# NIFTy-PPL/NIFTy

Hardware: AMD Instinct MI355X
Metric: MGVI iters/sec on 1024^3 RGSpace CorrelatedField, 8 samples; achieved HBM GB/s (higher is better)
Workload: dtype f32

## Files before the change

include/niftyk.h:

```cpp
#ifndef NIFTYK_H
#define NIFTYK_H
#include <stddef.h>
#include <stdint.h>

#ifdef __cplusplus
extern "C" {
#endif

typedef enum {
  NK_OK = 0,
  NK_ERR_INVALID = -1,
  NK_ERR_UNSUPPORTED = -2,
  NK_ERR_RUNTIME = -3,
  NK_ERR_NOMEM = -4
} nk_status;

typedef enum { NK_F32 = 0, NK_F64 = 1 } nk_dtype;

#define NK_HARTLEY_NON_CANONICAL 0
#define NK_HARTLEY_CANONICAL 1

enum { NK_PRO_PLAIN = 0, NK_PRO_AMP = 1, NK_PRO_AMP_JVP = 2, NK_PRO_MUL = 3 };
enum { NK_EPI_AFFINE = 0, NK_EPI_MUL = 1, NK_EPI_VJP = 2, NK_EPI_LIKELIHOOD = 3, NK_EPI_NONLIN = 4 };
enum { NK_LH_GAUSS = 0, NK_LH_POISSON = 1 };
// ... 110 lines not shown
typedef struct nk_tiled_csr {
  int64_t n_rows, n_slots;
  int32_t n_items, ny, nx, th, tw;
  const int32_t* item_tile;
  const int64_t* item_blk;
  const int32_t* blk_slot;
  const int64_t* row_slot;
  const uint16_t* loc;
  const float* wgt;
} nk_tiled_csr;
int nk_tiled_rowsum(const nk_tiled_csr* m, int count, const void* const* x, void* const* y, double* scratch, int dtype,
                    void* stream);

int nk_roll(int ndim, const int64_t* shape, const int64_t* shift, int elem_bytes, const void* in, void* out, void* stream);

int nk_bluestein_rows(int64_t rows, int n, int m, const void* in, const void* w, const void* bhat_br, const void* tw, void* out,
                      double scale, int in_real, int out_hartley, int dtype, void* stream);

int nk_cumsum(int64_t n, const void* in, void* out, int reverse, int dtype, void* stream);

int nk_cplx_rows(int64_t rows, int64_t in_cols, int64_t out_cols, const void* a, const void* w, void* out, int mode,
                 double scale, int sgn, int dtype, void* stream);

int nk_fold_copies(int64_t n, int copies, int64_t stride, const double* src, double* dst, void* stream);

int nk_octant_expand(int ndim, const int64_t* shape, const void* table, const int32_t* pidx, void* field, int dtype,
                     int compact, void* stream);
int nk_octant_scatter(int ndim, const int64_t* shape, const double* w8, const int32_t* pidx, double* abar,
                      int merge_swapped_lines, void* stream);
int nk_octant_expand_k2(int ndim, const int64_t* shape, const double* table, const int32_t* bin_k2, int64_t nb, void* dense,
                        void* field8, int dtype, const int32_t* line_order, void* stream);
int nk_octant_scatter_k2(int ndim, const int64_t* shape, const double* w8, const int32_t* pidx, const int32_t* bin_k2,
                         int64_t nb, double* scratch, double* abar, const double* w8max, void* stream);
int nk_segment_sum(int64_t nseg, const int32_t* rowptr, const int32_t* perm, const double* src, double* dst, int accumulate,
                   void* stream);
int nk_plan_octant_vjp(const nk_plan* plan);

int nk_pindex_from_k2(int ndim, const int64_t* shape, const int32_t* k2table, int32_t* pidx, int64_t* rho,
                      void* stream);

int nk_cg_curv(int64_t n, const void* d, const void* q, int dtype, double* scal, int accumulate, void* stream);
int nk_cg_update(int64_t n, void* x, void* r, const void* d, const void* q, const void* b, int dtype,
                 double* scal, int accumulate, void* stream);
int nk_cg_update_dr(int64_t n, void* x, void* r, const void* d, const void* q, int dtype, double* scal, int accumulate,
                    void* stream);
int nk_cg_direction(int64_t n, void* d, const void* r, int dtype, double* scal, int roll, void* stream);

typedef struct nk_product {
  int nsub;
  int64_t size[3];
  const int32_t* pidx[3];
  const double* tab[3];
  const double* dtab[3];
  const double* scale;
  const double* dscale;
} nk_product;
int nk_product_field(const nk_product* p, int tangent, void* out, int dtype, void* stream);
int nk_mirror_combine(int ndim, const int64_t* shape, const int* group, int nsub, const double* coef, const void* in,
                      void* out, double scale, double offset, int dtype, void* stream);
size_t nk_product_marginal_scratch(const nk_product* p, int which);
int nk_product_marginal(const nk_product* p, int which, const double* w, double* scratch, double* marg, void* stream);

int nk_amp_forward(int nb, const double* geo, const double* hyp, const double* lat, double* state, double* amp,
                   void* stream);
int nk_amp_jvp(int nb, const double* geo, const double* hyp, const double* lat, double* state, const double* dlat,
               double* damp, void* stream);
// ... 91 lines not shown
```

nifty_amd/_lib.py:

```python
import ctypes
import os

_HERE = os.path.dirname(os.path.abspath(__file__))
LIB_PATH = os.environ.get("NK_LIB_PATH") or os.path.join(_HERE, "csrc", "libniftyk.so")

NK_OK, NK_ERR_INVALID, NK_ERR_UNSUPPORTED, NK_ERR_RUNTIME, NK_ERR_NOMEM = 0, -1, -2, -3, -4
NK_F32, NK_F64 = 0, 1
PRO_PLAIN, PRO_AMP, PRO_AMP_JVP, PRO_MUL = 0, 1, 2, 3
EPI_AFFINE, EPI_MUL, EPI_VJP, EPI_LIKELIHOOD, EPI_NONLIN = 0, 1, 2, 3, 4
LH_GAUSS, LH_POISSON = 0, 1
NL_ID, NL_EXP, NL_SIGMOID = 0, 1, 2
OP_ADD, OP_SUB, OP_MUL, OP_DIV = 0, 1, 2, 3

_vp, _i, _i64, _d, _sz = ctypes.c_void_p, ctypes.c_int, ctypes.c_int64, ctypes.c_double, ctypes.c_size_t


class Fuse(ctypes.Structure):

    _fields_ = [
        ("pro", _i), ("in_", _vp), ("in2", _vp), ("pidx", _vp), ("amp", _vp), ("damp", _vp),
        ("epi", _i), ("out", _vp), ("scale", _d), ("offset", _d), ("mul", _vp), ("mul_scalar", _d),
        ("xi", _vp), ("addend", _vp), ("addend_scale", _d), ("accumulate", _i), ("abar", _vp), ("lh_kind", _i), ("nonlin", _i), ("data", _vp),
        ("icov", _vp), ("icov_scalar", _d), ("out2", _vp), ("value", _vp),
        ("afield", _vp), ("dampT", _vp), ("abar_copies", _i), ("abar_stride", _i64), ("dafield", _vp), ("w8", _vp),
# ... 44 lines not shown
    "nk_hartley_sandwich_pair": (_i, [_vp, ctypes.POINTER(Fuse), ctypes.POINTER(Fuse), _d, _i, _vp, _vp, _vp]),
    "nk_hartley_sandwich_group": (_i, [_vp, ctypes.POINTER(Fuse), _i, _d, _i, _vp, _vp]),
    "nk_group_order": (_i, [_i64, _i, ctypes.POINTER(_i64), ctypes.POINTER(_i64)]),
    "nk_group_grid_size": (_i64, [_i64, _i]),
    "nk_fftn": (_i, [_vp, _vp, _vp, _i, _d, _vp, _vp]),
    "nk_plan_c2c_ok": (_i, [_vp]),
    "nk_plan_c2c_lds": (_i, [_vp, ctypes.POINTER(_i64)]),
    "nk_profile_enable": (_i, [_i]),
    "nk_profile_collect": (_i, [_vp, _vp]),
    "nk_vdot": (_i, [_i64, _vp, _vp, _i, _vp, _i, _vp]),
    "nk_product_field": (_i, [ctypes.POINTER(Product), _i, _vp, _i, _vp]),
    "nk_mirror_combine": (_i, [_i, ctypes.POINTER(_i64), ctypes.POINTER(_i), _i, ctypes.POINTER(_d), _vp, _vp, _d, _d, _i, _vp]),
    "nk_product_marginal_scratch": (_sz, [ctypes.POINTER(Product), _i]),
    "nk_product_marginal": (_i, [ctypes.POINTER(Product), _i, _vp, _vp, _vp, _vp]),
    "nk_red_unit": (_i64, [_i64, _i]),
    "nk_red_layout": (_i, [_i64, _i, _i, _i, _i, _i, _vp]),
    "nk_red_finish": (_i, [_vp, _i, _i, _vp, _i, _vp]),
    "nk_sum": (_i, [_i64, _vp, _i, _vp, _i, _vp]),
    "nk_stats": (_i, [_i64, _vp, _i, _vp, _vp]),
    "nk_binary": (_i, [_i, _i64, _vp, _d, _vp, _d, _vp, _i, _vp]),
    "nk_cplx_muldiv": (_i, [_i64, _vp, _i, _d, _d, _vp, _i, _d, _d, _i, _i, _vp, _i, _vp]),
    "nk_cplx_pointwise": (_i, [_i, _i64, _vp, _vp, _i, _vp]),
    "nk_axpby": (_i, [_i64, _d, _vp, _d, _vp, _vp, _i, _vp]),
    "nk_axpby_sqnorm": (_i, [_i64, _d, _vp, _d, _vp, _vp, _i, _vp, _i, _vp]),
    "nk_pointwise": (_i, [_i, _d, _i64, _vp, _vp, _vp, _i, _vp]),
    "nk_clip": (_i, [_d, _d, _i64, _vp, _vp, _vp, _i, _vp]),
    "nk_gather": (_i, [_i64, _vp, _vp, _vp, _i, _vp]),
    "nk_scatter_add": (_i, [_i64, _vp, _vp, _i64, _vp, _i, _vp]),
    "nk_octant_expand": (_i, [_i, ctypes.POINTER(_i64), _vp, _vp, _vp, _i, _i, _vp]),
    "nk_octant_scatter": (_i, [_i, ctypes.POINTER(_i64), _vp, _vp, _vp, _i, _vp]),
    "nk_octant_expand_k2": (_i, [_i, ctypes.POINTER(_i64), _vp, _vp, _i64, _vp, _vp, _i, _vp, _vp]),
    "nk_segment_sum": (_i, [_i64, _vp, _vp, _vp, _vp, _i, _vp]),
    "nk_octant_scatter_k2": (_i, [_i, ctypes.POINTER(_i64), _vp, _vp, _vp, _i64, _vp, _vp, _vp, _vp]),
    "nk_plan_octant_vjp": (_i, [_vp]),
    "nk_fold_copies": (_i, [_i64, _i, _i64, _vp, _vp, _vp]),
    "nk_cumsum": (_i, [_i64, _vp, _vp, _i, _i, _vp]),
    "nk_cplx_rows": (_i, [_i64, _i64, _i64, _vp, _vp, _vp, _i, _d, _i, _i, _vp]),
    "nk_csr_rowsum": (_i, [_i64, _vp, _vp, _vp, _vp, _vp, _i, _i, _vp]),
    "nk_tiled_rowsum": (_i, [ctypes.POINTER(TiledCsr), _i, _vp, _vp, _vp, _i, _vp]),
    "nk_bluestein_rows": (_i, [_i64, _i, _i, _vp, _vp, _vp, _vp, _vp, _d, _i, _i, _i, _vp]),
    "nk_roll": (_i, [_i, ctypes.POINTER(_i64), ctypes.POINTER(_i64), _i, _vp, _vp, _vp]),
    "nk_spmv": (_i, [_i64, _vp, _vp, _vp, _vp, _vp, _i, _vp]),
    "nk_spmv_t": (_i, [_i64, _vp, _vp, _vp, _vp, _vp, _i, _vp]),
    "nk_pindex_from_k2": (_i, [_i, ctypes.POINTER(_i64), _vp, _vp, _vp, _vp]),
    "nk_cg_curv": (_i, [_i64, _vp, _vp, _i, _vp, _i, _vp]),
    "nk_cg_update": (_i, [_i64, _vp, _vp, _vp, _vp, _vp, _i, _vp, _i, _vp]),
    "nk_cg_update_dr": (_i, [_i64, _vp, _vp, _vp, _vp, _i, _vp, _i, _vp]),
    "nk_pcg64_normal_scratch_bytes": (_i64, [_i64, _i]),
    "nk_pcg64_normal": (_i, [_vp, _vp, _i64, _d, _d, _vp, _i, _vp, _i64, _i, _vp, _vp]),
    "nk_pcg64_fixed_scratch_bytes": (_i64, []),
    "nk_pcg64_uniform": (_i, [_vp, _vp, _i64, _d, _d, _vp, _i, _vp, _vp]),
    "nk_pcg64_pm1": (_i, [_vp, _vp, _i64, _vp, _i, _i, _vp, _vp]),
    "nk_pcg64_integers_scratch_bytes": (_i64, [_i64]),
    "nk_pcg64_integers": (_i, [_vp, _vp, _i64, _i64, ctypes.c_uint64, _i64, _vp, _vp, _vp, _vp]),
    "nk_cg_direction": (_i, [_i64, _vp, _vp, _i, _vp, _i, _vp]),
    "nk_amp_forward": (_i, [_i, _vp, _vp, _vp, _vp, _vp, _vp]),
    "nk_amp_jvp": (_i, [_i, _vp, _vp, _vp, _vp, _vp, _vp, _vp]),
    "nk_amp_vjp": (_i, [_i, _vp, _vp, _vp, _vp, _vp, _vp, _vp]),
    "nk_nufft_spread": (_i, [ctypes.POINTER(NufftPlan), _vp, _vp, _vp, _i, _vp]),
    "nk_nufft_interp": (_i, [ctypes.POINTER(NufftPlan), _vp, _vp, _i, _vp]),
    "nk_nufft_crop": (_i, [ctypes.POINTER(NufftPlan), _vp, _vp, _i, _vp]),
    "nk_nufft_pad": (_i, [ctypes.POINTER(NufftPlan), _vp, _i, _vp, _i, _vp]),
    "nk_sample_times": (_i, [ctypes.POINTER(SamplePlan), _vp, _vp, _i, _vp]),
    "nk_sample_adjoint": (_i, [ctypes.POINTER(SamplePlan), _vp, _vp, _vp, _i, _vp]),
    "nk_regrid_times": (_i, [_i64, _i64, _i64, _i64, _vp, _vp, _vp, _i, _vp, _i, _vp]),
    "nk_regrid_adjoint": (_i, [_i64, _i64, _i64, _i64, _vp, _vp, _vp, _i, _vp, _i, _vp]),
# ... 66 lines not shown
```

nifty_amd/csrc/nk_vec.hip:

```cpp
#include <hip/hip_runtime.h>

#include <algorithm>
#include <cfloat>

#include <cstdint>
#include <cstdlib>
#include <type_traits>

#include "nk_core.h"
#include "nk_util.h"

static constexpr int NK_VEC_THREADS = 256;
static constexpr int NK_MAX_BLOCKS = 256 * 8;
static constexpr int NK_VEC_CHUNK = 4096;

template <typename F, typename = void>
struct NkChunkUnits {
  static constexpr int value = NK_VEC_CHUNK / NK_VEC_THREADS;
};
template <typename F>
struct NkChunkUnits<F, std::void_t<decltype(F::CHUNK_UNITS)>> {
  static constexpr int value = F::CHUNK_UNITS;
};
static inline int nk_vec_env_int(const char* name, int dflt) {
// ... 1669 lines not shown
  __syncthreads();
  const bool ok = finite && npoints < (1u << 18);
  double* dst = partial + (int64_t)s * pstride + bin0;
  for (int i = threadIdx.x; i < nbin; i += blockDim.x)
    dst[i] = ok ? (double)(long long)acc[i] * inv : __longlong_as_double(0x7ff8000000000000LL);
}

extern "C" int nk_octant_scatter_k2(int ndim, const int64_t* shape, const double* w8, const int32_t* pidx,
                                    const int32_t* bin_k2, int64_t nb, double* scratch, double* abar, const double* w8max,
                                    void* stream) {
  NkOct o;
  int rc = nk_make_oct(ndim, shape, o);
  if (rc != NK_OK) return rc;
  if (!w8 || !pidx || !bin_k2 || !scratch || !abar || nb < 1 || nb > 0x7fffffff)
    return nk_set_error(NK_ERR_INVALID, "nk_octant_scatter_k2: bad argument");
  if ((int64_t)(o.Ah - 1) * (o.Ah - 1) + (int64_t)(o.Mh - 1) * (o.Mh - 1) + (int64_t)(o.Ch - 1) * (o.Ch - 1) >= (1 << 24))
    return nk_set_error(NK_ERR_UNSUPPORTED, "nk_octant_scatter_k2: k^2 range too large");
  const int64_t shells = (nb + NK_SHELL_BINS - 1) / NK_SHELL_BINS;
  const int64_t pstride = (nb + 31) / 32 * 32;
  static const int fp_atomics = nk_vec_env_int("NK_SCATTER_FP_ATOMICS", 0);
  const bool fixed = w8max != nullptr && !fp_atomics &&
                     (int64_t)o.Ah * o.Mh * o.Ch / NK_SHELL_SPLITS < ((int64_t)1 << 16) * shells;
  if (fixed)
    hipLaunchKernelGGL(k_octant_scatter_k2_fx, dim3((unsigned)(shells * NK_SHELL_SPLITS)), dim3(256), 0, (hipStream_t)stream, o,
                       w8, pidx, bin_k2, (int)nb, pstride, scratch, w8max);
  else
    hipLaunchKernelGGL(k_octant_scatter_k2, dim3((unsigned)(shells * NK_SHELL_SPLITS)), dim3(256), 0, (hipStream_t)stream, o, w8,
                       pidx, bin_k2, (int)nb, pstride, scratch);
  rc = nk_check_launch("k_octant_scatter_k2");
  if (rc != NK_OK) return rc;
  return nk_fold_copies(nb, NK_SHELL_SPLITS, pstride, scratch, abar, stream);
}

template <typename T, int LANES>
__global__ void __launch_bounds__(256) k_csr_rowsum(int64_t nrows, const int64_t* __restrict__ rowptr,
                                                    const int32_t* __restrict__ col, const float* __restrict__ wgt,
                                                    const T* __restrict__ x, T* __restrict__ y) {
  const int64_t gid = (int64_t)blockIdx.x * blockDim.x + threadIdx.x;
  const int64_t row = gid / LANES;
  const int lane = (int)(gid % LANES);
  int64_t lo = 0, hi = 0;
  if (row < nrows) lo = rowptr[row], hi = rowptr[row + 1];
  double acc = 0.0;
  if (wgt) {
    for (int64_t j = lo + lane; j < hi; j += LANES) acc += (double)wgt[j] * (double)x[col[j]];
  } else {
    for (int64_t j = lo + lane; j < hi; j += LANES) acc += (double)x[col[j]];
  }
#pragma unroll
  for (int off = LANES / 2; off > 0; off >>= 1) acc += __shfl_down(acc, off, LANES);
  if (lane == 0 && row < nrows) y[row] = (T)acc;
}

template <typename T>
__global__ void k_spmv_t(int64_t nrows, const int64_t* __restrict__ rowptr, const int32_t* __restrict__ col,
                         const float* __restrict__ wgt, const T* __restrict__ y, double* __restrict__ x) {
  const int lane = threadIdx.x & 63;
  const int64_t row = (int64_t)blockIdx.x * (blockDim.x >> 6) + (threadIdx.x >> 6);
  if (row >= nrows) return;
  const int64_t lo = rowptr[row], hi = rowptr[row + 1];
  const double yv = (double)y[row];
  for (int64_t j = lo + lane; j < hi; j += 64) atomicAdd(x + col[j], (double)wgt[j] * yv);
}


template <int MB>
// ... 417 lines not shown
```

nifty_amd/engine.py:

```python
import contextlib
import ctypes
import math
import os
import threading

import numpy as np
import torch

from . import _lib as L
from . import backend as B
from . import batched, parallel, random
from .domains import PowerSpace, RGSpace
from .minimization import ConjugateGradient, Energy, QuadraticEnergy

SMALL_KEYS = ("asperity", "flexibility", "fluctuations", "loglogavgslope", "zeromode")
LATENT_KEYS = ("asperity", "flexibility", "fluctuations", "loglogavgslope", "spectrum", "xi", "zeromode")
_NONLIN = {None: L.NL_ID, "": L.NL_ID, "exp": L.NL_EXP, "sigmoid": L.NL_SIGMOID}
SPECTRUM_DEVICE_DRAW_MAX_POINTS = int(os.environ.get("NK_SPECTRUM_DEVICE_DRAW_MAX_POINTS", str(1 << 25)))


def lognormal_moments(mean, sigma):
    checked = {}
    for name, value in (("mean", mean), ("sig", sigma)):
        checked[name] = float(value)
# ... 230 lines not shown
        return LatentVec(B.axpby(float(a), self.xi), B.axpby(float(a), self.small))

    __rmul__ = __mul__

    def __neg__(self):
        return self * (-1.0)

    def axpy(self, a, x):
        return x._lin(float(a), self, 1.0)

    def dot_device(self, o, result=None):
        res = B.vdot(self.xi.reshape(-1), o.xi.reshape(-1), result=result, accumulate=result is not None)
        return B.vdot(self.small, o.small, result=res, accumulate=True)

    def s_vdot(self, o):
        return float(self.dot_device(o).item())

    def norm(self, ord=2):
        if ord != 2:
            raise NotImplementedError
        return math.sqrt(self.s_vdot(self))


class _Dest:

    __slots__ = ("xi", "accumulate", "carries", "small", "after", "fresh")

    def __init__(self, xi, accumulate=False, carries=(), small=None, after=(), fresh=False):
        self.xi, self.accumulate, self.carries, self.small, self.after, self.fresh = xi, accumulate, carries, small, after, fresh


class _ScratchSet:

    __slots__ = ("damp", "dafield", "w8", "w8max", "workspace")

    def __init__(self, damp, dafield, w8, w8max, workspace):
        self.damp, self.dafield, self.w8, self.w8max, self.workspace = damp, dafield, w8, w8max, workspace


class _PairTree:

    MAX_CARRIES = 2

    def __init__(self, out, scratch):
        self._stack = []
        self._first = out
        self._pool = scratch
        self._free = []

    def place(self, last, small=None):
        size, joined = 1, []
        while self._stack and (last or self._stack[-1][0] == size):
            n, t = self._stack.pop()
            joined.append(t)
            size += n
        if not joined:
            t = self._first if self._first is not None else (self._free.pop() if self._free else self._pool())
            self._first = None
            self._stack.append((1, t))
            return _Dest(t, small=small, fresh=True)
        ride = joined[:self.MAX_CARRIES] if len(joined) > 1 else []
        target = joined[len(ride)] if len(joined) > len(ride) else None
        if target is None:
            target, ride = ride[-1], ride[:-1]
        rest = joined[len(ride) + 1:]
        after, inner = [], target
        for t in rest:
            after.append((t, inner))
            inner = t
        self._free += ride + ([target] + rest[:-1] if rest else [])
# ... 76 lines not shown
            self.abar = torch.zeros(nb, dtype=torch.float64, device=self.device)
            self.damp = torch.empty(nb, dtype=torch.float64, device=self.device)
            self.latbar = torch.empty(self.nsmall, dtype=torch.float64, device=self.device)
            self.tmp = torch.empty(self.shape, dtype=dtype, device=self.device)
            self.octant_vjp = bool(L.load().nk_plan_octant_vjp(self.plan.handle))
            sw = os.environ.get("NK_SANDWICH", "1")
            self.sandwich = (self.octant_vjp and B.plan_sandwich(self.plan) and sw != "0"
                             and (len(self.shape) == 3 or sw == "2"))
            self.fused_direction = self.sandwich and os.environ.get("NK_CG_FUSED_DIRECTION", "1") != "0"
            oct_n = int(np.prod([n // 2 + 1 for n in self.shape]))
            self.field_shape = (oct_n,) if self.octant_vjp else self.shape
            self.pidx8 = None
            if self.octant_vjp:
                osl = tuple(slice(0, n // 2 + 1) for n in self.shape)
                self.pidx8 = self.pidx.view(self.shape)[osl].contiguous().reshape(-1)
            self.dafield = torch.empty(self.field_shape, dtype=dtype, device=self.device)
            self.w8 = torch.empty(oct_n, dtype=torch.float64, device=self.device) if self.octant_vjp else None
            self.w8max = torch.zeros(1, dtype=torch.float64, device=self.device)
            self.merge_swapped = int(len(self.shape) == 3 and self.shape[0] == self.shape[1]
                                     and hsp.distances[0] == hsp.distances[1])
            self.bin_k2 = None
            self.seg_plan = None
            if self.octant_vjp and len(self.shape) == 3 and ps._data.get("k2table") is not None and max(self.shape) >= 64:
                k2 = np.nonzero(hsp._k2_flags())[0].astype(np.int32)
                if len(k2) == nb and int(k2[-1]) < (1 << 24):
                    self.bin_k2 = torch.from_numpy(k2).to(self.device)
            self.scatter_fixed_point = False
            if self.bin_k2 is not None:
                a_idx = torch.arange(self.shape[0] // 2 + 1, device=self.device, dtype=torch.int64)
                key = (self.pidx8.view(self.shape[0] // 2 + 1, -1) // 4096).to(torch.int64) * 16 + (a_idx % 16)[:, None]
                self.scatter_busiest = int(torch.bincount(key.reshape(-1)).max().item())
                self.scatter_fixed_point = self.scatter_busiest < (1 << 18)
                del key, a_idx
            self.k2_dense = self.k2_line_order = None
            if self.bin_k2 is not None and os.environ.get("NK_EXPAND_K2", "1") != "0":
                self.k2_dense = torch.zeros(int(self.bin_k2[-1].item()) + 1, dtype=dtype, device=self.device)
                if len(self.shape) == 3 and os.environ.get("NK_EXPAND_ORDER", "1") != "0":
                    a2 = torch.arange(self.shape[0] // 2 + 1, device=self.device, dtype=torch.int64) ** 2
                    b2 = torch.arange(self.shape[1] // 2 + 1, device=self.device, dtype=torch.int64) ** 2
                    self.k2_line_order = torch.argsort((a2[:, None] + b2[None, :]).reshape(-1), stable=True).to(torch.int32)
            if self.octant_vjp and self.bin_k2 is None and os.environ.get("NK_SEGMENT_SUM", "1") != "0":
                self.seg_plan = B.bin_plan(self.pidx8, self.nb)
            self.wide = (dtype == torch.float32 and self.octant_vjp and os.environ.get("NK_WIDE_FORWARD", "1") != "0")
            self.wide_generic = (dtype == torch.float32 and not self.octant_vjp
                                 and os.environ.get("NK_WIDE_FORWARD", "1") != "0")
            self._wide_state = None
            if (not self.octant_vjp and self.N <= B.BIN_PLAN_MAX and os.environ.get("NK_SEGMENT_SUM", "1") != "0"):
                self.full_plan = B.bin_plan(self.pidx, self.nb)
                self.wfull = torch.empty(self.N, dtype=torch.float64, device=self.device)
        if likelihood not in ("gaussian", "poisson"):
            raise ValueError("likelihood must be 'gaussian' or 'poisson'")
        self.lh_kind = L.LH_GAUSS if likelihood == "gaussian" else L.LH_POISSON
        self.nonlin = _NONLIN[nonlin]
        self.icov_field, self.icov_scalar = None, 1.0
        self.response = response
        self.wide_response = False
        self.data_shape = self.shape if response is None else (int(response.n_data),)
        if response is not None:
            if int(response.n_pix) != self.N:
                raise ValueError("response does not act on this grid")
            if getattr(response, "grid_shape", 0) is None:
                response.grid_shape = tuple(self.shape)
            self.sandwich = self.fused_direction = False
            self.wide_response = self.wide or self.wide_generic
            self.wide = self.wide_generic = False
        if data is not None:
# ... 102 lines not shown
            f.abar, f.w8 = self.abar.data_ptr(), sc.w8.data_ptr()
            if self.scatter_fixed_point:
                f.w8max = sc.w8max.data_ptr()
        elif self.full_plan is not None:
            f.abar, f.wfull = self.abar.data_ptr(), self.wfull.data_ptr()
        else:
            f.abar, f.abar_copies, f.abar_stride = self.abar_priv.data_ptr(), self.abar_copies, self.abar_stride

    def _amp_tangent(self, lp, d, sc, gather=False):
        L.check(L.load().nk_amp_jvp(self.nb, self.geo.data_ptr(), self.hyp.data_ptr(), lp.x.small.data_ptr(),
                                    lp.state.data_ptr(), d.small.data_ptr(), sc.damp.data_ptr(), B._stream()), "nk_amp_jvp")
        if gather:
            return sc.damp if self.tdtype == torch.float64 else sc.damp.to(self.tdtype)
        self._amp_field(sc.damp, out=sc.dafield)

    def _bin_sums(self, sc):
        shp = (ctypes.c_int64 * len(self.shape))(*self.shape)
        if self.bin_k2 is not None:
            L.check(L.load().nk_octant_scatter_k2(len(self.shape), shp, sc.w8.data_ptr(), self.pidx.data_ptr(),
                                                  self.bin_k2.data_ptr(), self.nb, self.scatter_scratch.data_ptr(),
                                                  self.abar.data_ptr(),
                                                  sc.w8max.data_ptr() if self.scatter_fixed_point else 0, B._stream()),
                    "nk_octant_scatter_k2")
        elif self.seg_plan is not None:
            rowptr, perm, lanes = self.seg_plan
            L.check(L.load().nk_csr_rowsum(self.nb, rowptr.data_ptr(), perm.data_ptr(), 0, sc.w8.data_ptr(),
                                           self.abar.data_ptr(), L.NK_F64, lanes, B._stream()), "nk_csr_rowsum")
        else:
            self.abar.zero_()
            L.check(L.load().nk_octant_scatter(len(self.shape), shp, sc.w8.data_ptr(), self.pidx.data_ptr(),
                                               self.abar.data_ptr(), self.merge_swapped, B._stream()),
                    "nk_octant_scatter")

    def scratch_sets(self, count):
        more = self.__dict__.setdefault("_more_sets", [])
        while 1 + len(more) < count:
            more.append(_ScratchSet(torch.empty_like(self.damp), torch.empty_like(self.dafield), torch.empty_like(self.w8),
                                    torch.zeros_like(self.w8max), torch.empty_like(self.plan.workspace)))
        return [_ScratchSet(self.damp, self.dafield, self.w8, self.w8max, self.plan.workspace)] + more[:count - 1]

    def release_group_buffers(self):
        del self.__dict__.get("_more_sets", [])[1:]

    def _forward_nonlin(self, xi, amp, afield, out, out2):
        f = self._fuse()
        self._pro_amp(f, xi, amp, afield)
        self._epi_nonlin(f, out, out2)
        B.hartley_fused(self.plan, f)
        self._count("transforms", 1)

    def signal(self, x, want_derivative=False):
        amp, _ = self._amp_forward(x.small)
        afield = self._amp_field(amp)
        out = torch.empty(self.shape, dtype=self.tdtype, device=self.device)
        d = torch.empty_like(out) if want_derivative else None
        self._forward_nonlin(x.xi, amp, afield, out, d)
        return (out, d) if want_derivative else out

    def _vjp(self, lp, w, scale, addend, addend_scale, accumulate, out_xi, dot_out=None, w2=None, sandwich=None, carries=()):
        f = self._fuse()
        sc = self.scratch_sets(1)[0]
        if dot_out is not None and (addend is None or not self.octant_vjp):
            raise ValueError("dot_out needs an addend and the register-resident transform pipeline")
        if sandwich is not None:
            sandwich[0](f)
            f.mul, f.mul_scalar = B.ptr(sandwich[2]), sandwich[3]
        else:
            f.pro, f.in_ = L.PRO_PLAIN, w.data_ptr()
            if w2 is not None:
                f.pro, f.in2 = L.PRO_MUL, w2.data_ptr()
        self._epi_vjp(f, lp, sc, out_xi, scale, addend, addend_scale, accumulate, carries, dot_out)
        if not self.octant_vjp and self.full_plan is None:
            self.abar_priv.zero_()
        if sandwich is None:
            B.hartley_fused(self.plan, f)
        else:
            B.hartley_sandwich(self.plan, f, sandwich[1])
        if self.octant_vjp:
            self._bin_sums(sc)
        elif self.full_plan is not None:
            rowptr, perm, lanes = self.full_plan
            L.check(L.load().nk_csr_rowsum(self.nb, rowptr.data_ptr(), perm.data_ptr(), 0, self.wfull.data_ptr(),
                                           self.abar.data_ptr(), L.NK_F64, lanes, B._stream()), "nk_csr_rowsum")
        else:
            L.check(L.load().nk_fold_copies(self.nb, self.abar_copies, self.abar_stride, self.abar_priv.data_ptr(),
                                            self.abar.data_ptr(), B._stream()), "nk_fold_copies")
        self._count("transforms", 1 if sandwich is None else 2)

    def _amp_vjp(self, lp):
        L.check(L.load().nk_amp_vjp(self.nb, self.geo.data_ptr(), self.hyp.data_ptr(), lp.x.small.data_ptr(),
                                    lp.state.data_ptr(), self.abar.data_ptr(), self.latbar.data_ptr(), B._stream()),
                "nk_amp_vjp")

    def metric_point(self, x):
        if self.response is None and self.const_mid:
            lp = LinPoint()
            lp.x = x
            lp.amp, lp.state = self._amp_forward(x.small)
            lp.afield = self._amp_field(lp.amp)
            lp.mid_scalar = self.icov_scalar
            return lp
        return self.linearize(x, want_gradient=False)

    def linearize(self, x, grad_acc=None, n_total=1, value_acc=None, dest=None, want_gradient=True):
        lp = LinPoint()
        lp.x = x
        lp.amp, lp.state = self._amp_forward(x.small)
        lp.afield = self._amp_field(lp.amp)
        w = 1.0 / n_total
        value = torch.zeros(1, dtype=torch.float64, device=self.device) if value_acc is None else value_acc
        lhval = torch.zeros(1, dtype=torch.float64, device=self.device)
        if self.response is not None:
            return self._linearize_response(lp, x, grad_acc if dest is None else dest, w, value, lhval, want_gradient)
        f = self._fuse()
        self._pro_amp(f, x.xi, lp.amp, lp.afield)
        gs = self.tmp
        if not self.const_mid:
            lp.mid = torch.empty(self.shape, dtype=self.tdtype, device=self.device)
        else:
            lp.mid_scalar = self.icov_scalar
        self._epi_likelihood(f, gs, lp.mid, lhval)
        if self.wide:
            plan64, afield64, dense64 = self._wide_buffers()
            f.afield, f.io32 = self._amp_field(lp.amp, out=afield64, dense=dense64).data_ptr(), 1
# ... 179 lines not shown
        else:
            self._jvp_field(lp, d, sc, lp.mid, lp.mid_scalar, self.tmp)
            self._vjp(lp, self.tmp, scale, avec.xi if afac else None, afac, dot_out=dot_out, **where)
        self._finish_metric(lp, avec, out, first, afac, dest)

    def pair_ready(self):
        return bool(self.sandwich and self.octant_vjp and self.response is None and self.bin_k2 is not None
                    and len(self.shape) == 3 and self.const_mid and os.environ.get("NK_PAIR_FINAL", "1") != "0")

    def lh_metric_accumulate_pair(self, lpa, lpb, d, out, scale, first, identity=0.0, dot_out=None, cg_direction=None,
                                  dests=None, identity_first=0.0):
        if cg_direction is not None and not self.fused_direction:
            raise ValueError("cg_direction needs the sandwich pipeline (FusedModel.fused_direction)")
        sets = self.scratch_sets(2)
        if dests is None:
            dests = (_Dest(out.xi, accumulate=not first), _Dest(out.xi, accumulate=True))
        members = ((lpa, sets[0], dests[0], identity_first, cg_direction, None, first),
                   (lpb, sets[1], dests[1], identity, None, dot_out if identity else None, False))
        fuses = []
        for lp, sc, dest, ident, direction, dot, _ in members:
            self._amp_tangent(lp, d, sc)
            f = self._fuse()
            self._pro_amp_jvp(f, lp, d, sc, cg_direction=direction)
            f.mul, f.mul_scalar = B.ptr(lp.mid), lp.mid_scalar
            self._epi_vjp(f, lp, sc, dest.xi, scale, d.xi if ident else None, ident, dest.accumulate, dest.carries, dot)
            fuses.append(f)
        if dot_out is not None and not identity:
            raise ValueError("dot_out needs the identity term (the addend of the epilogue)")
        B.hartley_sandwich_pair(self.plan, fuses[0], fuses[1], self.h_dvol, sets[1].workspace)
        _PairTree.settle(dests[1])
        if cg_direction is not None:
            cg_direction[1].roll()
        self._count("transforms", 4)
        for lp, sc, dest, ident, _, _, is_first in members:
            self._bin_sums(sc)
            self._finish_metric(lp, d, out, is_first, ident, dest)

    def group_ready(self):
        return bool(self.pair_ready() and self.fused_direction and os.environ.get("NK_GROUP", "1") != "0"
                    and os.environ.get("NK_DA_GATHER", "0") != "1")

    def lh_metric_group(self, lp, jobs):
        sets = self.scratch_sets(len(jobs))
        fuses, outs, adds = [], [], []
        points = [job.get("lp", lp) for job in jobs]
        for job, sc, lp in zip(jobs, sets, points):
            d = job["d"]
            avec, afac = (d, job.get("identity", 0.0)) if job.get("addend") is None else job["addend"]
            out = LatentVec(torch.empty_like(d.xi), None)
            self._amp_tangent(lp, d, sc)
            f = self._fuse()
            self._pro_amp_jvp(f, lp, d, sc, cg_direction=job.get("cg_direction"))
            f.mul, f.mul_scalar = B.ptr(lp.mid), lp.mid_scalar
            if job.get("dot_out") is not None and not afac:
                raise ValueError("dot_out needs an addend and the register-resident transform pipeline")
            self._epi_vjp(f, lp, sc, out.xi, 1.0, avec.xi if afac else None, afac, dot_out=job.get("dot_out"))
            fuses.append(f)
            outs.append(out)
            adds.append((avec, afac))
        B.hartley_sandwich_group(self.plan, fuses, self.h_dvol, [sc.workspace for sc in sets])
        for job, sc, out, (avec, afac), lp in zip(jobs, sets, outs, adds, points):
            self._count("transforms", 2)
            self._bin_sums(sc)
            if job.get("cg_direction") is not None:
                job["cg_direction"][1].roll()
            self._finish_metric(lp, avec, out, True, afac, _Dest(out.xi, accumulate=False))
        return outs

    def _finish_metric(self, lp, d, out, first, identity, dest=None):
        self._amp_vjp(lp)
        if dest is not None:
            _PairTree.settle(dest)
            if dest.small is not None:
                dest.small.append(B.axpby(1.0, self.latbar, identity, d.small) if identity else B.axpby(1.0, self.latbar))
                self._count("metric", 1)
                return
        if first:
            out.small = B.axpby(1.0, self.latbar, identity, d.small) if identity else B.axpby(1.0, self.latbar)
        else:
            B.axpby(1.0, self.latbar, 1.0, out.small, out=out.small)
            if identity:
                B.axpby(identity, d.small, 1.0, out.small, out=out.small)
        self._count("metric", 1)

    def metric(self, lp, d, dot_out=None, cg_direction=None):
        out = LatentVec(torch.empty_like(d.xi), None)
        self.lh_metric_accumulate(lp, d, out, 1.0, True, identity=1.0, dot_out=dot_out, cg_direction=cg_direction)
        return out

    def lh_metric(self, lp, d, minus=None):
        out = LatentVec(torch.empty_like(d.xi), None)
        self.lh_metric_accumulate(lp, d, out, 1.0, True, addend=None if minus is None else (minus, -1.0))
        return out

    def trafo_point(self, x):
        lp = LinPoint()
        lp.x = x
        lp.amp, lp.state = self._amp_forward(x.small)
        lp.afield = self._amp_field(lp.amp)
        if self.response is not None:
            lp.gp = torch.empty(self.shape, dtype=self.tdtype, device=self.device)
            self._forward_nonlin(x.xi, lp.amp, lp.afield, self.tmp, lp.gp)
            mu = self.response.times(self.tmp)
# ... 869 lines not shown
```

Before: 0.2183.

## Batch octant k2 shell scatter across group members in one kernel

Adds a grouped octant scatter kernel that processes 2 or 4 members' w8 arrays in one launch. The bin index table and loop traversal are shared, and each member gets its own fixed-point shared-memory accumulator. Scratch sets now own separate abar and scatter buffers, so the metric group and pair paths can call one grouped scatter instead of one per member. The aim is to cut repeated pidx/bin_k2 reads and launch count. The cost is more shared memory per block and more register pressure, which may reduce occupancy.

```diff
diff --git a/include/niftyk.h b/include/niftyk.h
--- a/include/niftyk.h
+++ b/include/niftyk.h
@@ -166,6 +166,9 @@
                         void* field8, int dtype, const int32_t* line_order, void* stream);
 int nk_octant_scatter_k2(int ndim, const int64_t* shape, const double* w8, const int32_t* pidx, const int32_t* bin_k2,
                          int64_t nb, double* scratch, double* abar, const double* w8max, void* stream);
+int nk_octant_scatter_k2_group(int ndim, const int64_t* shape, int n, const double* const* w8, const int32_t* pidx,
+                               const int32_t* bin_k2, int64_t nb, double* const* scratch, double* const* abar,
+                               const double* const* w8max, void* stream);
 int nk_segment_sum(int64_t nseg, const int32_t* rowptr, const int32_t* perm, const double* src, double* dst, int accumulate,
                    void* stream);
 int nk_plan_octant_vjp(const nk_plan* plan);
diff --git a/nifty_amd/_lib.py b/nifty_amd/_lib.py
--- a/nifty_amd/_lib.py
+++ b/nifty_amd/_lib.py
@@ -100,6 +100,7 @@
     "nk_octant_expand_k2": (_i, [_i, ctypes.POINTER(_i64), _vp, _vp, _i64, _vp, _vp, _i, _vp, _vp]),
     "nk_segment_sum": (_i, [_i64, _vp, _vp, _vp, _vp, _i, _vp]),
     "nk_octant_scatter_k2": (_i, [_i, ctypes.POINTER(_i64), _vp, _vp, _vp, _i64, _vp, _vp, _vp, _vp]),
+    "nk_octant_scatter_k2_group": (_i, [_i, ctypes.POINTER(_i64), _i, _vp, _vp, _vp, _i64, _vp, _vp, _vp, _vp]),
     "nk_plan_octant_vjp": (_i, [_vp]),
     "nk_fold_copies": (_i, [_i64, _i, _i64, _vp, _vp, _vp]),
     "nk_cumsum": (_i, [_i64, _vp, _vp, _i, _i, _vp]),
diff --git a/nifty_amd/csrc/nk_vec.hip b/nifty_amd/csrc/nk_vec.hip
--- a/nifty_amd/csrc/nk_vec.hip
+++ b/nifty_amd/csrc/nk_vec.hip
@@ -1725,6 +1725,196 @@
   return nk_fold_copies(nb, NK_SHELL_SPLITS, pstride, scratch, abar, stream);
 }
 
+#ifndef NK_SHELL_GROUP_BINS
+#define NK_SHELL_GROUP_BINS 4096
+#endif
+#ifndef NK_SHELL_GROUP_THREADS2
+#define NK_SHELL_GROUP_THREADS2 512
+#endif
+#ifndef NK_SHELL_GROUP_THREADS4
+#define NK_SHELL_GROUP_THREADS4 1024
+#endif
+#ifndef NK_SHELL_GROUP_MAX
+#define NK_SHELL_GROUP_MAX 4
+#endif
+#define NK_SCATTER_GROUP_LIMIT 4
+
+template <int G>
+struct NkShellGroup {
+  const double* w8[G];
+  const double* w8max[G];
+  double* partial[G];
+};
+
+template <int G, int BINS, int THREADS>
+__global__ void __launch_bounds__(THREADS)
+    k_octant_scatter_k2_fx_g(NkOct o, int n, NkShellGroup<G> m, const int32_t* __restrict__ pidx,
+                             const int32_t* __restrict__ bin_k2, int nb, int64_t pstride) {
+  __shared__ unsigned long long acc[G * BINS];
+  __shared__ unsigned int npoints;
+  const int j = blockIdx.x / NK_SHELL_SPLITS, s = blockIdx.x % NK_SHELL_SPLITS;
+  const int bin0 = j * BINS;
+  const int nbin = min(BINS, nb - bin0);
+  for (int i = threadIdx.x; i < G * BINS; i += THREADS) acc[i] = 0ull;
+  if (threadIdx.x == 0) npoints = 0u;
+  __syncthreads();
+  double scale[G], inv[G];
+  bool finite[G];
+#pragma unroll
+  for (int g = 0; g < G; ++g) {
+    const double gmax = g < n ? *m.w8max[g] : 0.0;
+    finite[g] = gmax <= 1.79769313486231570815e308;
+    int e = 0;
+    if (finite[g] && gmax > 0.0) (void)frexp(gmax, &e);
+    e = max(e, -979);
+    scale[g] = ldexp(1.0, 44 - e), inv[g] = ldexp(1.0, e - 44);
+  }
+  unsigned int mine = 0u;
+  const int klo = bin_k2[bin0];
+  const int khi = bin0 + BINS < nb ? bin_k2[bin0 + BINS] : 0x7fffffff;
+  const int hc2 = (o.Ch - 1) * (o.Ch - 1);
+  constexpr int LINES = THREADS / 16, NU = G == 4 ? NK_SHELL_NU / 2 : NK_SHELL_NU * 3 / 4;
+  const int grp = threadIdx.x >> 4, l16 = threadIdx.x & 15;
+  const bool last = khi == 0x7fffffff;
+  for (int a = s; a < o.Ah; a += NK_SHELL_SPLITS) {
+    const int ra = a * a;
+    if (ra >= khi) break;
+    const int b_hi = last ? o.Mh : min(o.Mh, nk_isqrt_ceil(khi - ra));
+    const int b_lo = nk_isqrt_ceil(klo - hc2 - ra);
+    for (int b0 = b_lo + grp; b0 < b_hi; b0 += LINES * NU) {
+      int cc[NU], ce[NU];
+      int64_t wo[NU];
+      const int32_t* pl[NU];
+      double v[G][NU];
+      int32_t pb[NU];
+      const int64_t wo0 = ((int64_t)a * o.Mh + b0) * o.Ch;
+      const int32_t* pl0 = pidx + ((int64_t)a * o.M + b0) * o.NL;
+      const int64_t wstep = (int64_t)LINES * o.Ch, pstep = (int64_t)LINES * o.NL;
+      int r2 = ra + b0 * b0, dr2 = 2 * LINES * b0 + LINES * LINES;
+#pragma unroll
+      for (int u = 0; u < NU; ++u) {
+        const int b = b0 + u * LINES;
+        const bool on = b < b_hi;
+        cc[u] = nk_isqrt_ceil(klo - r2) + l16;
+        ce[u] = on ? (last ? o.Ch : min(o.Ch, nk_isqrt_ceil(khi - r2))) : 0;
+        wo[u] = wo0 + u * wstep;
+        pl[u] = pl0 + u * pstep;
+        const bool in = cc[u] < ce[u];
+        pb[u] = in ? pl[u][cc[u]] : bin0;
+#pragma unroll
+        for (int g = 0; g < G; ++g) v[g][u] = (in && g < n) ? m.w8[g][wo[u] + cc[u]] : 0.0;
+        r2 += dr2;
+        dr2 += 2 * LINES * LINES;
+      }
+#pragma unroll
+      for (int u = 0; u < NU; ++u)
+        if (cc[u] < ce[u]) {
+#pragma unroll
+          for (int g = 0; g < G; ++g)
+            if (g < n) atomicAdd(&acc[g * BINS + pb[u] - bin0], nk_fixed_rn(v[g][u] * scale[g]));
+          ++mine;
+        }
+#pragma unroll
+      for (int u = 0; u < NU; ++u)
+        for (int c = cc[u] + 16; c < ce[u]; c += 16) {
+          const int bin = pl[u][c] - bin0;
+#pragma unroll
+          for (int g = 0; g < G; ++g)
+            if (g < n) atomicAdd(&acc[g * BINS + bin], nk_fixed_rn(m.w8[g][wo[u] + c] * scale[g]));
+          ++mine;
+        }
+    }
+  }
+  atomicAdd(&npoints, mine);
+  __syncthreads();
+  const bool few = npoints < (1u << 18);
+#pragma unroll
+  for (int g = 0; g < G; ++g) {
+    if (g >= n) break;
+    const bool ok = finite[g] && few;
+    double* dst = m.partial[g] + (int64_t)s * pstride + bin0;
+    for (int i = threadIdx.x; i < nbin; i += THREADS)
+      dst[i] = ok ? (double)(long long)acc[g * BINS + i] * inv[g] : __longlong_as_double(0x7ff8000000000000LL);
+  }
+}
+
+template <int G, int BINS, int THREADS>
+static void nk_launch_shell_group(const NkOct& o, int n, const NkShellGroup<G>& m, const int32_t* pidx, const int32_t* bin_k2,
+                                  int64_t nb, int64_t pstride, hipStream_t st) {
+  const int64_t shells = (nb + BINS - 1) / BINS;
+  hipLaunchKernelGGL((k_octant_scatter_k2_fx_g<G, BINS, THREADS>), dim3((unsigned)(shells * NK_SHELL_SPLITS)), dim3(THREADS), 0,
+                     st, o, n, m, pidx, bin_k2, (int)nb, pstride);
+}
+
+template <int G>
+static int nk_shell_group_launch(const NkOct& o, int n, const double* const* w8, const double* const* w8max,
+                                 double* const* scratch, const int32_t* pidx, const int32_t* bin_k2, int64_t nb, int64_t pstride,
+                                 int bins, int threads, hipStream_t st) {
+  NkShellGroup<G> m;
+  for (int g = 0; g < G; ++g) {
+    const int k = g < n ? g : 0;
+    m.w8[g] = w8[k], m.w8max[g] = w8max[k], m.partial[g] = scratch[k];
+  }
+#define NK_SHELL_GROUP_CASE(B, T) \
+  if (bins == B && threads == T) nk_launch_shell_group<G, B, T>(o, n, m, pidx, bin_k2, nb, pstride, st); else
+  NK_SHELL_GROUP_CASE(4096, 512) NK_SHELL_GROUP_CASE(4096, 1024) NK_SHELL_GROUP_CASE(4096, 256)
+  NK_SHELL_GROUP_CASE(2048, 512) NK_SHELL_GROUP_CASE(2048, 1024) NK_SHELL_GROUP_CASE(2048, 256)
+  return nk_set_error(NK_ERR_INVALID, "nk_octant_scatter_k2_group: NK_SHELL_GROUP_BINS is 2048 or 4096, NK_SHELL_GROUP_THREADS 0, 256, 512 or 1024");
+#undef NK_SHELL_GROUP_CASE
+  return nk_check_launch("k_octant_scatter_k2_fx_g");
+}
+
+extern "C" int nk_octant_scatter_k2_group(int ndim, const int64_t* shape, int n, const double* const* w8, const int32_t* pidx,
+                                          const int32_t* bin_k2, int64_t nb, double* const* scratch, double* const* abar,
+                                          const double* const* w8max, void* stream) {
+  NkOct o;
+  int rc = nk_make_oct(ndim, shape, o);
+  if (rc != NK_OK) return rc;
+  if (n < 1 || n > NK_SCATTER_GROUP_LIMIT) return nk_set_error(NK_ERR_INVALID, "nk_octant_scatter_k2_group: 1 <= n <= 4");
+  if (!w8 || !pidx || !bin_k2 || !scratch || !abar || nb < 1 || nb > 0x7fffffff)
+    return nk_set_error(NK_ERR_INVALID, "nk_octant_scatter_k2_group: bad argument");
+  bool scaled = w8max != nullptr;
+  for (int g = 0; g < n; ++g) {
+    if (!w8[g] || !scratch[g] || !abar[g]) return nk_set_error(NK_ERR_INVALID, "nk_octant_scatter_k2_group: null member array");
+    for (int h = 0; h < g; ++h)
+      if (scratch[h] == scratch[g] || abar[h] == abar[g])
+        return nk_set_error(NK_ERR_INVALID, "nk_octant_scatter_k2_group: members share a scratch or an output array");
+    scaled = scaled && w8max[g] != nullptr;
+  }
+  if ((int64_t)(o.Ah - 1) * (o.Ah - 1) + (int64_t)(o.Mh - 1) * (o.Mh - 1) + (int64_t)(o.Ch - 1) * (o.Ch - 1) >= (1 << 24))
+    return nk_set_error(NK_ERR_UNSUPPORTED, "nk_octant_scatter_k2_group: k^2 range too large");
+  static const int fp_atomics = nk_vec_env_int("NK_SCATTER_FP_ATOMICS", 0);
+  static const int bins = nk_vec_env_int("NK_SHELL_GROUP_BINS", NK_SHELL_GROUP_BINS);
+  static const int threads_env = nk_vec_env_int("NK_SHELL_GROUP_THREADS", 0);
+  static const int gmax = nk_vec_env_int("NK_SHELL_GROUP_MAX", NK_SHELL_GROUP_MAX);
+  const int64_t points = (int64_t)o.Ah * o.Mh * o.Ch / NK_SHELL_SPLITS;
+  const int64_t shells_g = (nb + (bins > 0 ? bins : NK_SHELL_GROUP_BINS) - 1) / (bins > 0 ? bins : NK_SHELL_GROUP_BINS);
+  const int64_t shells_1 = (nb + NK_SHELL_BINS - 1) / NK_SHELL_BINS;
+  const bool fixed = scaled && !fp_atomics && points < ((int64_t)1 << 16) * shells_g && points < ((int64_t)1 << 16) * shells_1;
+  const int64_t pstride = (nb + 31) / 32 * 32;
+  for (int g0 = 0; g0 < n;) {
+    const int left = n - g0;
+    const int take = !fixed || left == 1 || gmax < 2 ? 1 : (gmax >= 4 ? left : 2);
+    if (take == 1) {
+      rc = nk_octant_scatter_k2(ndim, shape, w8[g0], pidx, bin_k2, nb, scratch[g0], abar[g0], w8max ? w8max[g0] : nullptr, stream);
+      if (rc != NK_OK) return rc;
+    } else {
+      const int threads = threads_env > 0 ? threads_env : (take == 2 ? NK_SHELL_GROUP_THREADS2 : NK_SHELL_GROUP_THREADS4);
+      rc = take == 2 ? nk_shell_group_launch<2>(o, take, w8 + g0, w8max + g0, scratch + g0, pidx, bin_k2, nb, pstride, bins, threads,
+                                                (hipStream_t)stream)
+                     : nk_shell_group_launch<4>(o, take, w8 + g0, w8max + g0, scratch + g0, pidx, bin_k2, nb, pstride, bins, threads,
+                                                (hipStream_t)stream);
+      if (rc != NK_OK) return rc;
+      for (int g = g0; g < g0 + take; ++g) {
+        rc = nk_fold_copies(nb, NK_SHELL_SPLITS, pstride, scratch[g], abar[g], stream);
+        if (rc != NK_OK) return rc;
+      }
+    }
+    g0 += take;
+  }
+  return NK_OK;
+}
+
 template <typename T, int LANES>
 __global__ void __launch_bounds__(256) k_csr_rowsum(int64_t nrows, const int64_t* __restrict__ rowptr,
                                                     const int32_t* __restrict__ col, const float* __restrict__ wgt,
diff --git a/nifty_amd/engine.py b/nifty_amd/engine.py
--- a/nifty_amd/engine.py
+++ b/nifty_amd/engine.py
@@ -286,10 +286,11 @@
 
 class _ScratchSet:
 
-    __slots__ = ("damp", "dafield", "w8", "w8max", "workspace")
-
-    def __init__(self, damp, dafield, w8, w8max, workspace):
+    __slots__ = ("damp", "dafield", "w8", "w8max", "workspace", "abar", "scatter_scratch")
+
+    def __init__(self, damp, dafield, w8, w8max, workspace, abar, scatter_scratch):
         self.damp, self.dafield, self.w8, self.w8max, self.workspace = damp, dafield, w8, w8max, workspace
+        self.abar, self.scatter_scratch = abar, scatter_scratch
 
 
 class _PairTree:
@@ -432,6 +433,7 @@
                 self.scatter_busiest = int(torch.bincount(key.reshape(-1)).max().item())
                 self.scatter_fixed_point = self.scatter_busiest < (1 << 18)
                 del key, a_idx
+            self.group_scatter = self.scatter_fixed_point and os.environ.get("NK_GROUP_SCATTER", "1") != "0"
             self.k2_dense = self.k2_line_order = None
             if self.bin_k2 is not None and os.environ.get("NK_EXPAND_K2", "1") != "0":
                 self.k2_dense = torch.zeros(int(self.bin_k2[-1].item()) + 1, dtype=dtype, device=self.device)
@@ -600,12 +602,32 @@
                                                self.abar.data_ptr(), self.merge_swapped, B._stream()),
                     "nk_octant_scatter")
 
+    def _bin_sums_group(self, sets):
+        if not self.group_scatter or len(sets) < 2:
+            return False
+        shp = (ctypes.c_int64 * len(self.shape))(*self.shape)
+
+        def ptrs(ts):
+            return (ctypes.c_void_p * len(ts))(*[t.data_ptr() for t in ts])
+
+        L.check(L.load().nk_octant_scatter_k2_group(len(self.shape), shp, len(sets), ptrs([sc.w8 for sc in sets]),
+                                                    self.pidx.data_ptr(), self.bin_k2.data_ptr(), self.nb,
+                                                    ptrs([sc.scatter_scratch for sc in sets]), ptrs([sc.abar for sc in sets]),
+                                                    ptrs([sc.w8max for sc in sets]), B._stream()),
+                "nk_octant_scatter_k2_group")
+        return True
+
     def scratch_sets(self, count):
         more = self.__dict__.setdefault("_more_sets", [])
         while 1 + len(more) < count:
+            own = self.group_scatter
             more.append(_ScratchSet(torch.empty_like(self.damp), torch.empty_like(self.dafield), torch.empty_like(self.w8),
-                                    torch.zeros_like(self.w8max), torch.empty_like(self.plan.workspace)))
-        return [_ScratchSet(self.damp, self.dafield, self.w8, self.w8max, self.plan.workspace)] + more[:count - 1]
+                                    torch.zeros_like(self.w8max), torch.empty_like(self.plan.workspace),
+                                    torch.zeros_like(self.abar) if own else self.abar,
+                                    torch.empty(16 * (self.nb + 32), dtype=torch.float64, device=self.device) if own
+                                    else self.scatter_scratch))
+        return [_ScratchSet(self.damp, self.dafield, self.w8, self.w8max, self.plan.workspace, self.abar,
+                            self.scatter_scratch)] + more[:count - 1]
 
     def release_group_buffers(self):
         del self.__dict__.get("_more_sets", [])[1:]
@@ -655,9 +677,10 @@
                                             self.abar.data_ptr(), B._stream()), "nk_fold_copies")
         self._count("transforms", 1 if sandwich is None else 2)
 
-    def _amp_vjp(self, lp):
+    def _amp_vjp(self, lp, abar=None):
+        abar = self.abar if abar is None else abar
         L.check(L.load().nk_amp_vjp(self.nb, self.geo.data_ptr(), self.hyp.data_ptr(), lp.x.small.data_ptr(),
-                                    lp.state.data_ptr(), self.abar.data_ptr(), self.latbar.data_ptr(), B._stream()),
+                                    lp.state.data_ptr(), abar.data_ptr(), self.latbar.data_ptr(), B._stream()),
                 "nk_amp_vjp")
 
     def metric_point(self, x):
@@ -903,9 +926,11 @@
         if cg_direction is not None:
             cg_direction[1].roll()
         self._count("transforms", 4)
+        together = self._bin_sums_group(sets)
         for lp, sc, dest, ident, _, _, is_first in members:
-            self._bin_sums(sc)
-            self._finish_metric(lp, d, out, is_first, ident, dest)
+            if not together:
+                self._bin_sums(sc)
+            self._finish_metric(lp, d, out, is_first, ident, dest, abar=sc.abar if together else None)
 
     def group_ready(self):
         return bool(self.pair_ready() and self.fused_direction and os.environ.get("NK_GROUP", "1") != "0"
@@ -930,16 +955,18 @@
             outs.append(out)
             adds.append((avec, afac))
         B.hartley_sandwich_group(self.plan, fuses, self.h_dvol, [sc.workspace for sc in sets])
+        together = self._bin_sums_group(sets)
         for job, sc, out, (avec, afac), lp in zip(jobs, sets, outs, adds, points):
             self._count("transforms", 2)
-            self._bin_sums(sc)
+            if not together:
+                self._bin_sums(sc)
             if job.get("cg_direction") is not None:
                 job["cg_direction"][1].roll()
-            self._finish_metric(lp, avec, out, True, afac, _Dest(out.xi, accumulate=False))
+            self._finish_metric(lp, avec, out, True, afac, _Dest(out.xi, accumulate=False), abar=sc.abar if together else None)
         return outs
 
-    def _finish_metric(self, lp, d, out, first, identity, dest=None):
-        self._amp_vjp(lp)
+    def _finish_metric(self, lp, d, out, first, identity, dest=None, abar=None):
+        self._amp_vjp(lp, abar)
         if dest is not None:
             _PairTree.settle(dest)
             if dest.small is not None:
```

Result: faster. 0.2206, median of 6 (+1.0%).
